# VISION-SJTU/UniDefense

Measured on AMD Instinct MI355X. Metric: images/sec fwd+bwd (256x256, EffNet-b4), higher is better.
Workload: dtype f32

## Files before the change

include/unidefense_hip.h:

```cpp
#ifndef UNIDEFENSE_HIP_H
#define UNIDEFENSE_HIP_H
#include <stdint.h>

#ifdef __cplusplus
extern "C" {
#endif

#define UD_EINVAL (-1000)

typedef void* ud_stream_t;

typedef struct {
    int N, Hin, Win, Cin, Hout, Wout, KH, KW, stride, pad_t, pad_l, transposed;
} ud_conv_geom;

typedef struct {
    const float* A; const float* B; float* C;
    int M, N, K;
    long lda, ldb, ldc;
    int a_mode, b_mode, out_mode, split_k;
    int batch; long strideA, strideB, strideC;
    ud_conv_geom g;
    double* stat_sum; double* stat_sumsq;
    int half_mask;
// ... 393 lines not shown
int ud_pj_bwd_fused_a(const float* d, const float* dp, const ud_bn_ref* bn, const float* s, const float* w, int N, int HW, int CE,
                      int CO, float* dw, double* dgate, float* part, ud_stream_t stream);
int ud_pj_bwd_fused_b(const float* d, const float* dp, const ud_bn_ref* bn, const float* s, const float* dpool, float inv_hw,
                      const float* w, int N, int HW, int CE, int CO, float* dz, double* s1, double* s2, ud_stream_t stream);
int ud_normbwd_apply_plane_half(const void* x, const void* dy, const float* keep, float inv_keep, const ud_bn_ref* bn,
                                int dy_is_dz, const double* s1, const double* s2, const double* s1_local,
                                const double* s2_local, int G, int R, int C, uint16_t* plane, long panel_stride,
                                float* inv_scale, float* dgamma, float* dbeta, ud_stream_t stream);
int ud_se_bwd_a(const double* dgate, const float* s2, const float* s1, const float* We, double* ds1_acc, float* dWe,
                float* dbe, int N, int C, int Cs, ud_stream_t stream);
int ud_se_bwd_b(const double* ds1_acc, const float* s1, const float* Wr, const double* pool, float pool_scale,
                float* dpool, float* dWr, float* dbr, int N, int C, int Cs, ud_stream_t stream);
int ud_se_scale_bwd_bn(const void* dc, const void* x, const ud_bn_ref* bn, const float* s, const float* dpool,
    float inv_hw, void* dz, double* s1, double* s2, double* ws, int G, int R, int C, int f16, ud_stream_t
    stream);
long ud_coldot_bn_eval_ws_doubles(int G, int R, int C);
int ud_coldot_bn_eval(const void* dy, const void* x, const ud_bn_ref* bn, int G, int R, int C, double* out, double* ws,
                      int f16, ud_stream_t stream);
int ud_se_scale_bwd_bn_eval(const void* dc, const void* x, const ud_bn_ref* bn, const float* s, const float* dpool,
                            float inv_hw, void* dd, int G, int R, int C, int f16, ud_stream_t stream);
int ud_bn_eval_bwd(const void* dy, const void* x, const ud_bn_ref* bn, void* dx, int G, int R, int C, int f16,
                   ud_stream_t stream);
int ud_normbwd_apply_mix(const void* x, const void* dz, const ud_bn_ref* bn, const double* s1, const double* s2,
    const double* s1_local, const double* s2_local, const void* diff, int G, int R, int C, void* dd,
    double* dalpha_acc, float* dgamma, float* dbeta, double* energy, int f16, ud_stream_t stream);
int ud_gate_grad_from_acc(const double* acc, const float* alpha, float* out, ud_stream_t stream);
int ud_bn_apply(const void* x, const ud_bn_ref* bn, void* y, int G, int R, int C, int f16, ud_stream_t stream);
int ud_dwconv_bwd_data_bn(const void* dy, const float* gate_alpha, int gate_mode, const float* wt, const void*
    add, const void* x, const ud_bn_ref* bn, void* dz, double* s1, double* s2, double* ws, int N, int H, int W,
    int C, int Ho, int Wo, int K, int stride, int pad_t, int pad_l, int f16, ud_stream_t stream);
// ... 80 lines not shown
```

unidefense_amd/csrc/fused.hip:

```cpp
#include "bnref.h"

namespace {

struct Rows {
    int r, r_end;
    long idx, step;
};
__device__ __forceinline__ Rows rows_of(const RedGeom& q, int ri, int c4) {
    Rows w;
    const int g = blockIdx.z, p = blockIdx.x;
    const int r_begin = p * q.rows_per_chunk;
    w.r_end = r_begin + q.rows_per_chunk;
    if (w.r_end > q.R) w.r_end = q.R;
    w.step = (long)q.rpi * q.C4;
    w.r = r_begin + ri;
    w.idx = (long)g * q.R * q.C4 + (long)w.r * q.C4 + c4;
    return w;
}

__device__ __forceinline__ bool is_updater(int ri) { return blockIdx.x == 0 && blockIdx.z == 0 && ri == 0; }

template <int NQ>
__device__ __forceinline__ void red_out(const RedGeom& q, int ri, bool active, int c4, double (&v)[8], double* a1,
                                        double* a2, double* part, bool per_group) {
// ... 2 lines not shown
    if (part) {
        const long o = (((long)blockIdx.z * q.P + blockIdx.x) * q.C4 + c4) * 4;
        const long plane = (long)q.G * q.P * q.C4 * 4;
#pragma unroll
        for (int e = 0; e < 4; ++e) {
            part[o + e] = v[e];
            if (NQ == 8) part[plane + o + e] = v[4 + e];
        }
    } else {
        const long o = ((long)(per_group ? blockIdx.z : 0) * q.C4 + c4) * 4;
#pragma unroll
        for (int e = 0; e < 4; ++e) {
            atomic_add_f64(a1 + o + e, v[e]);
            if (NQ == 8) atomic_add_f64(a2 + o + e, v[4 + e]);
        }
    }
}

template <typename T>
__global__ __launch_bounds__(NT) void colstats_kernel(RedGeom q, const T* __restrict__ x, double* __restrict__ sum,
                                                      double* __restrict__ sumsq, double* __restrict__ part) {
    int ri, c4;
    const bool active = thread_coords(q, ri, c4);
    const In4<T> x4{x};
    double v[8] = {0, 0, 0, 0, 0, 0, 0, 0};
    if (active) {
        Rows w = rows_of(q, ri, c4);
        for (; w.r + 3 * q.rpi < w.r_end; w.r += 4 * q.rpi, w.idx += 4 * w.step) {
            f32x4 a0 = x4[w.idx], a1 = x4[w.idx + w.step], a2 = x4[w.idx + 2 * w.step], a3 = x4[w.idx + 3 * w.step];
#pragma unroll
// ... 42 lines not shown
                });
            } else {
                const In4<T> in[1] = {x4};
                for_rows<T, 1>(w.r, w.r_end, q.rpi, w.idx, w.step, in, fin, [&](long, int, const f32x4(&t)[1]) UD_LAMBDA_INLINE {
                    const f32x4 a = bn_apply<ACT>(t[0], cb);
#pragma unroll
                    for (int e = 0; e < 4; ++e) v[e] += (double)a[e];
                    mo = fmaxf(mo, fmaxf(fmaxf(fabsf(a[0]), fabsf(a[1])), fmaxf(fabsf(a[2]), fabsf(a[3]))));
                });
            }
        });
        if (!DOT && is_updater(ri)) bn_update_running(bn, blockIdx.z, q.C4, c4);
    }
    red_out<4>(q, ri, active, c4, v, out, nullptr, part, true);
    if (!DOT) ud_absmax_commit(mo, amax);
}

__global__ __launch_bounds__(NT) void fc_fwd_d_kernel(const double* __restrict__ xsum, float xscale,
                                                      const float* __restrict__ W, const float* __restrict__ b,
                                                      float* __restrict__ y, int N, int I, int O) {
    const int wave = (blockIdx.x * NT + threadIdx.x) >> 6, lane = threadIdx.x & 63;
    if (wave >= N * O) return;
    const int n = wave / O, o = wave % O;
    float acc = 0.f;
#pragma unroll 4
    for (int i = lane; i < I; i += 64) acc += ((float)xsum[(long)n * I + i] * xscale) * W[(long)o * I + i];
    acc = ud_wave_sum(acc);
    if (lane == 0) y[(long)n * O + o] = acc + (b ? b[o] : 0.f);
}

// ... 219 lines not shown
    const In4<T> in[1] = {In4<T>{x}};
    const Out4<T> y4{y};
    const BnRaw raw = bn_issue(bn, blockIdx.z, q.C4, c4);
    Bn4 cb;
    const Rows w = rows_of(q, ri, c4);
    auto fin = [&]() UD_LAMBDA_INLINE { cb = bn_finish(bn, raw); };
    act_switch(bn.act, [&](auto ac) UD_LAMBDA_INLINE {
        constexpr int ACT = decltype(ac)::value;
        for_rows<T, 1>(w.r, w.r_end, q.rpi, w.idx, w.step, in, fin,
                       [&](long idx, int, const f32x4(&t)[1]) UD_LAMBDA_INLINE { y4.st(idx, bn_apply<ACT>(t[0], cb)); });
    });
    if (is_updater(ri)) bn_update_running(bn, blockIdx.z, q.C4, c4);
}

constexpr int kDz = -1;
template <int MODE>
__device__ __forceinline__ void dz_terms(const f32x4& a, const f32x4& d, const Bn4& cb, float sc, f32x4& dz, f32x4& xh) {
#pragma unroll
    for (int e = 0; e < 4; ++e) {
        xh[e] = (a[e] - cb.mu[e]) * cb.is[e];
        float g = d[e];
        if (MODE != kDz) {
            g = mul_rn(g, sc);
            if (MODE) g = mul_rn(g, ud_act_grad_fast(cb.ga[e] * xh[e] + cb.be[e], MODE));
        }
        dz[e] = g;
    }
}
template <typename F>
__device__ __forceinline__ void dz_switch(int dy_is_dz, int act, F&& f) {
    if (dy_is_dz) f(ActC<kDz>{});
    else act_switch(act, f);
}

template <typename T>
__global__ __launch_bounds__(NT) void normbwd_sums_kernel(RedGeom q, const T* __restrict__ x,
                                                          const T* __restrict__ dy, const float* __restrict__ keep,
                                                          float inv_keep, ud_bn_ref bn, int dy_is_dz,
                                                          double* __restrict__ s1, double* __restrict__ s2,
                                                          double* __restrict__ s3, double* __restrict__ part) {
    int ri, c4;
    const bool active = thread_coords(q, ri, c4);
    const In4<T> x4{x}, d4{dy};
    double v[8] = {0, 0, 0, 0, 0, 0, 0, 0};
    f32x4 en = {0.f, 0.f, 0.f, 0.f};
    if (active) {
        const BnRaw raw = bn_issue(bn, blockIdx.z, q.C4, c4);
// ... 26 lines not shown
        if (active && ri == 0) {
#pragma unroll
            for (int e = 0; e < 4; ++e) atomic_add_f64(s3 + (long)c4 * 4 + e, ev[e]);
        }
    }
    red_out<8>(q, ri, active, c4, v, s1, s2, part, false);
}

struct PlanesDst {
    uint16_t* buf;
    long panel, plane;
    float* inv_scale;
    const double* energy;
};

template <typename T, bool MIX, int PL = 0>
__global__ __launch_bounds__(NT) void normbwd_apply_kernel(RedGeom q, const T* __restrict__ x,
                                                           const T* __restrict__ dy, const float* __restrict__ keep,
                                                           float inv_keep, ud_bn_ref bn, int dy_is_dz,
                                                           const double* __restrict__ s1, const double* __restrict__ s2,
                                                           const double* __restrict__ s1l, const double* __restrict__ s2l,
                                                           const T* __restrict__ freq,
                                                           T* __restrict__ dx, double* __restrict__ dalpha_acc,
                                                           float* __restrict__ dgamma, float* __restrict__ dbeta,
                                                           uint32_t* __restrict__ amax, double* __restrict__ energy,
                                                           PlanesDst pd) {
    int ri, c4;
    const bool active = thread_coords(q, ri, c4);
    BnRaw raw{};
    double t1d[4] = {0, 0, 0, 0}, t2d[4] = {0, 0, 0, 0};
    float kraw = 0.f;
    if (active) {
        raw = bn_issue(bn, blockIdx.z, q.C4, c4);
#pragma unroll
        for (int e = 0; e < 4; ++e) t1d[e] = s1[c4 * 4 + e];
#pragma unroll
        for (int e = 0; e < 4; ++e) t2d[e] = s2[c4 * 4 + e];
        if (keep) kraw = keep[blockIdx.z];
    }
    float ps = 1.f;
    if constexpr (PL == 2) {
        if (blockIdx.x == 0 && blockIdx.y == 0 && blockIdx.z == 0 && threadIdx.x == 0) *pd.inv_scale = 1.f;
    }
    if constexpr (PL == 1) {
        __shared__ float pl_red[NT / 64];
        float gm = 0.f;
        for (int i = threadIdx.x; i < q.C4 * 4; i += NT) {
            const double m = bn.sum[i] * bn.inv_count;
// ... 17 lines not shown
    double acc = 0.0;
    float mo = 0.f;
    f32x4 en = {0.f, 0.f, 0.f, 0.f};
    if (active) {
        Bn4 cb;
        float sc = 1.f;
        f32x4 t1, t2, k;
        const Rows w = rows_of(q, ri, c4);
        uint16_t* po = PL ? pd.buf + (long)(c4 >> 3) * pd.panel + (c4 & 7) * 4 : nullptr;
        const int npad = (PL && c4 == q.C4 - 1) ? 7 - (c4 & 7) : 0;
        const long prow0 = (long)blockIdx.z * q.R;
        auto fin = [&]() UD_LAMBDA_INLINE {
            cb = bn_finish(bn, raw);
            if (keep) sc = kraw * inv_keep;
            k = cb.ga * cb.is;
#pragma unroll
            for (int e = 0; e < 4; ++e) {
                t1[e] = (float)t1d[e] * (float)bn.inv_count;
                t2[e] = (float)t2d[e] * (float)bn.inv_count;
            }
        };
        auto row = [&](auto mc, const f32x4& a, const f32x4& d, const f32x4* f, long idx, int r) UD_LAMBDA_INLINE {
            constexpr int MODE = decltype(mc)::value;
            f32x4 dz, xh, o;
            dz_terms<MODE>(a, d, cb, sc, dz, xh);
#pragma unroll
            for (int e = 0; e < 4; ++e) o[e] = k[e] * __builtin_fmaf(-xh[e], t2[e], dz[e] - t1[e]);
            if constexpr (PL == 2) {
                typedef unsigned short u16x4 __attribute__((ext_vector_type(4)));
                const long prow = prow0 + r;
                Quad<T>::st(reinterpret_cast<T*>(po + prow * 32), 0, o);
                for (int z = 1; z <= npad; ++z) *reinterpret_cast<u16x4*>(po + prow * 32 + 4 * z) = u16x4{0, 0, 0, 0};
            } else if constexpr (PL == 1) {
                typedef unsigned short u16x4 __attribute__((ext_vector_type(4)));
                const long prow = prow0 + r;
                uint16_t h0[4], h1[4];
#pragma unroll
                for (int e = 0; e < 4; ++e) ud_split_h2(o[e] * ps, h0[e], h1[e]);
                *reinterpret_cast<u16x4*>(po + prow * 32) = u16x4{h0[0], h0[1], h0[2], h0[3]};
                *reinterpret_cast<u16x4*>(po + prow * 32 + pd.plane) = u16x4{h1[0], h1[1], h1[2], h1[3]};
                for (int z = 1; z <= npad; ++z) {
                    *reinterpret_cast<u16x4*>(po + prow * 32 + 4 * z) = u16x4{0, 0, 0, 0};
                    *reinterpret_cast<u16x4*>(po + prow * 32 + 4 * z + pd.plane) = u16x4{0, 0, 0, 0};
                }
            } else {
                o4.st(idx, o);
                mo = fmaxf(mo, fmaxf(fmaxf(fabsf(o[0]), fabsf(o[1])), fmaxf(fabsf(o[2]), fabsf(o[3]))));
                if constexpr (MIX) {
#pragma unroll
                    for (int e = 0; e < 4; ++e) acc += (double)ud_rounded<T>(o[e]) * (double)(*f)[e];
                    en += o * o;
                }
            }
        };
        dz_switch(dy_is_dz, bn.act, [&](auto mc) UD_LAMBDA_INLINE {
            if constexpr (MIX) {
                const In4<T> in[3] = {x4, d4, fr4};
                for_rows<T, 3>(w.r, w.r_end, q.rpi, w.idx, w.step, in, fin, [&](long idx, int r, const f32x4(&t)[3]) UD_LAMBDA_INLINE {
                    row(mc, t[0], t[1], &t[2], idx, r);
                });
            } else {
                const In4<T> in[2] = {x4, d4};
                for_rows<T, 2>(w.r, w.r_end, q.rpi, w.idx, w.step, in, fin, [&](long idx, int r, const f32x4(&t)[2]) UD_LAMBDA_INLINE {
                    row(mc, t[0], t[1], nullptr, idx, r);
                });
            }
        });
        if (is_updater(ri)) {
#pragma unroll
            for (int e = 0; e < 4; ++e) {
// ... 198 lines not shown
        __syncthreads();
        if (own) {
#pragma unroll 8
            for (int n = 0; n < nn; ++n) {
                const float g = sh[sl * IP + n];
                acc += g * ud_act_fast(s1[(long)(n0 + n) * Cs + i], 1);
                accb += g;
            }
        }
    }
    if (!own) return;
    dWe[(long)c * Cs + i] = acc;
    if (i == 0) dbe[c] = accb;
}

__global__ __launch_bounds__(NT) void se_bwd_b_kernel(const double* __restrict__ ds1_acc, const float* __restrict__ s1,
                                                      const float* __restrict__ Wr, const double* __restrict__ pool,
                                                      float pool_scale, float* __restrict__ dpool,
                                                      float* __restrict__ dWr, float* __restrict__ dbr, int N, int C,
                                                      int Cs) {
    __shared__ float sh[NT];
    const int c = blockIdx.x * NT + threadIdx.x;
    if ((int)blockIdx.y < N) {
        const int n = blockIdx.y;
        if ((int)threadIdx.x < Cs)
            sh[threadIdx.x] = (float)ds1_acc[(long)n * Cs + threadIdx.x] * ud_act_grad_fast(s1[(long)n * Cs + threadIdx.x], 1);
        __syncthreads();
        if (c >= C) return;
        float acc = 0.f;
#pragma unroll 8
        for (int i = 0; i < Cs; ++i) acc += sh[i] * Wr[(long)i * C + c];
        dpool[(long)n * C + c] = acc;
        return;
    }
    const int i = blockIdx.y - N;
    if ((int)threadIdx.x < N)
        sh[threadIdx.x] = (float)ds1_acc[(long)threadIdx.x * Cs + i] * ud_act_grad_fast(s1[(long)threadIdx.x * Cs + i], 1);
    __syncthreads();
    if (blockIdx.x == 0 && threadIdx.x == 0) {
        float b = 0.f;
        for (int n = 0; n < N; ++n) b += sh[n];
        dbr[i] = b;
    }
    if (c >= C) return;
    float acc = 0.f;
#pragma unroll 8
    for (int n = 0; n < N; ++n) acc += sh[n] * ((float)pool[(long)n * C + c] * pool_scale);
// ... 390 lines not shown
    return finish_reduce(pl, 2, false, C, ws, s1, s2, s);
}

int ud_normbwd_apply(const void* x, const void* dy, const float* keep, float inv_keep, const ud_bn_ref* bn,
                     int dy_is_dz, const double* s1, const double* s2, const double* s1_local,
                     const double* s2_local, int G, int R, int C, void* dx, float* dgamma, float* dbeta, int f16,
                     uint32_t* absmax, ud_stream_t stream) {
    if (ud_bn_eval_form(bn)) return UD_EINVAL;
    if (!shape_ok(G, R, C) || !x || !dy || !bn || !s1 || !s2 || !dx || bn->G != 1) return UD_EINVAL;
    if ((dgamma || dbeta) && (!s1_local || !s2_local)) return UD_EINVAL;
    RedGeom q = geom_ew(G, R, C);
    UD_STORAGE_DISPATCH(f16, hipLaunchKernelGGL((normbwd_apply_kernel<T, false>), red_grid(q), dim3(NT), 0,
                                                (hipStream_t)stream, q, (const T*)x, (const T*)dy, keep, inv_keep, *bn,
                                                dy_is_dz, s1, s2, s1_local, s2_local, (const T*)nullptr, (T*)dx,
                                                (double*)nullptr, dgamma, dbeta, absmax, (double*)nullptr,
                                                PlanesDst{nullptr, 0, 0, nullptr, nullptr}));
    UD_LAUNCH_CHECK();
    return 0;
}

int ud_normbwd_apply_planes(const float* x, const float* dy, const float* keep, float inv_keep, const ud_bn_ref* bn,
                            int dy_is_dz, const double* s1, const double* s2, const double* s1_local,
                            const double* s2_local, const double* energy, int G, int R, int C, uint16_t* planes,
                            long panel_stride, long plane_stride, float* inv_scale, float* dgamma, float* dbeta,
                            ud_stream_t stream) {
    if (ud_bn_eval_form(bn)) return UD_EINVAL;
    if (!shape_ok(G, R, C) || !x || !dy || !bn || !s1 || !s2 || !energy || !planes || !inv_scale || bn->G != 1 || !bn->gamma)
        return UD_EINVAL;
    if ((dgamma || dbeta) && (!s1_local || !s2_local)) return UD_EINVAL;
    const long rows = (long)G * R;
    if (panel_stride < 32 * rows || plane_stride < (long)ud_cdiv(C, 32) * panel_stride) return UD_EINVAL;
    RedGeom q = geom_ew(G, R, C);
    hipLaunchKernelGGL((normbwd_apply_kernel<float, false, 1>), red_grid(q), dim3(NT), 0, (hipStream_t)stream, q, x, dy, keep,
                       inv_keep, *bn, dy_is_dz, s1, s2, s1_local, s2_local, (const float*)nullptr, (float*)nullptr,
                       (double*)nullptr, dgamma, dbeta, (uint32_t*)nullptr, (double*)nullptr,
                       PlanesDst{planes, panel_stride, plane_stride, inv_scale, energy});
    UD_LAUNCH_CHECK();
    return 0;
}

int ud_normbwd_apply_plane_half(const void* x, const void* dy, const float* keep, float inv_keep, const ud_bn_ref* bn,
                                int dy_is_dz, const double* s1, const double* s2, const double* s1_local,
                                const double* s2_local, int G, int R, int C, uint16_t* plane, long panel_stride,
                                float* inv_scale, float* dgamma, float* dbeta, ud_stream_t stream) {
    if (ud_bn_eval_form(bn)) return UD_EINVAL;
    if (!shape_ok(G, R, C) || !x || !dy || !bn || !s1 || !s2 || !plane || !inv_scale || bn->G != 1) return UD_EINVAL;
    if ((dgamma || dbeta) && (!s1_local || !s2_local)) return UD_EINVAL;
    if (panel_stride < 32L * G * R) return UD_EINVAL;
    RedGeom q = geom_ew(G, R, C);
    hipLaunchKernelGGL((normbwd_apply_kernel<_Float16, false, 2>), red_grid(q), dim3(NT), 0, (hipStream_t)stream, q,
                       (const _Float16*)x, (const _Float16*)dy, keep, inv_keep, *bn, dy_is_dz, s1, s2, s1_local, s2_local,
                       (const _Float16*)nullptr, (_Float16*)nullptr, (double*)nullptr, dgamma, dbeta, (uint32_t*)nullptr,
                       (double*)nullptr, PlanesDst{plane, panel_stride, 0, inv_scale, nullptr});
    UD_LAUNCH_CHECK();
    return 0;
}

int ud_normbwd_apply_mix(const void* x, const void* dz, const ud_bn_ref* bn, const double* s1, const double* s2,
                         const double* s1_local, const double* s2_local, const void* diff, int G, int R, int C,
                         void* dd, double* dalpha_acc, float* dgamma, float* dbeta, double* energy, int f16,
                         ud_stream_t stream) {
    if (ud_bn_eval_form(bn)) return UD_EINVAL;
    if (!shape_ok(G, R, C) || !x || !dz || !bn || !s1 || !s2 || !dd || !diff || !dalpha_acc || bn->G != 1)
        return UD_EINVAL;
    if ((dgamma || dbeta) && (!s1_local || !s2_local)) return UD_EINVAL;
    RedGeom q = make_geom_ex(G, R, C, 512, 4096, 4);
    UD_STORAGE_DISPATCH(f16, hipLaunchKernelGGL((normbwd_apply_kernel<T, true>), red_grid(q), dim3(NT), 0,
                                                (hipStream_t)stream, q, (const T*)x, (const T*)dz, (const float*)nullptr,
                                                1.f, *bn, 1, s1, s2, s1_local, s2_local, (const T*)diff, (T*)dd,
                                                dalpha_acc, dgamma, dbeta, (uint32_t*)nullptr, energy,
                                                PlanesDst{nullptr, 0, 0, nullptr, nullptr}));
    UD_LAUNCH_CHECK();
    return 0;
}

int ud_gate_grad_from_acc(const double* acc, const float* alpha, float* out, ud_stream_t stream) {
    if (!acc || !alpha || !out) return UD_EINVAL;
    hipLaunchKernelGGL(gate_grad_from_acc_kernel, dim3(1), dim3(64), 0, (hipStream_t)stream, acc, alpha, out);
    UD_LAUNCH_CHECK();
    return 0;
}

int ud_se_bwd_a(const double* dgate, const float* s2, const float* s1, const float* We, double* ds1_acc, float* dWe,
                float* dbe, int N, int C, int Cs, ud_stream_t stream) {
    if (N < 1 || C < 1 || Cs < 1 || Cs > 128 || !dgate || !s2 || !s1 || !We || !ds1_acc || (!dWe != !dbe)) return UD_EINVAL;
    hipStream_t s = (hipStream_t)stream;
// ... 4 lines not shown
        hipLaunchKernelGGL(se_bwd_a_kernel<64>, grid, dim3(NT), 0, s, dgate, s2, s1, We, ds1_acc, dWe, dbe, N, C, Cs);
    } else {
        dim3 grid((unsigned)(role1 + (wg ? ud_cdiv(C, NT / 128) : 0)));
        hipLaunchKernelGGL(se_bwd_a_kernel<128>, grid, dim3(NT), 0, s, dgate, s2, s1, We, ds1_acc, dWe, dbe, N, C, Cs);
    }
    UD_LAUNCH_CHECK();
    return 0;
}

int ud_se_bwd_b(const double* ds1_acc, const float* s1, const float* Wr, const double* pool, float pool_scale,
                float* dpool, float* dWr, float* dbr, int N, int C, int Cs, ud_stream_t stream) {
    const bool wg = dWr != nullptr;
    if (N < 1 || N > NT || C < 1 || Cs < 1 || Cs > NT || !ds1_acc || !s1 || !Wr || !dpool || (!dWr != !dbr) || (wg && !pool))
        return UD_EINVAL;
    dim3 grid((unsigned)ud_cdiv(C, NT), (unsigned)(N + (wg ? Cs : 0)));
    hipLaunchKernelGGL(se_bwd_b_kernel, grid, dim3(NT), 0, (hipStream_t)stream, ds1_acc, s1, Wr, pool, pool_scale, dpool,
                       dWr, dbr, N, C, Cs);
    UD_LAUNCH_CHECK();
    return 0;
}

int ud_se_scale_bwd_bn(const void* dc, const void* x, const ud_bn_ref* bn, const float* s, const float* dpool,
                       float inv_hw, void* dz, double* s1, double* s2, double* ws, int G, int R, int C, int f16,
                       ud_stream_t stream) {
    if (ud_bn_eval_form(bn)) return UD_EINVAL;
    if (!shape_ok(G, R, C) || !dc || !x || !bn || !s || !dpool || !dz || !s1 || !s2 || bn->G != 1) return UD_EINVAL;
    hipStream_t st = (hipStream_t)stream;
    RedPlan pl = plan_reduce(G, R, C, false, ws);
    UD_STORAGE_DISPATCH(f16, hipLaunchKernelGGL(se_scale_bwd_bn_kernel<T>, red_grid(pl.q), dim3(NT), 0, st, pl.q,
                                                (const T*)dc, (const T*)x, *bn, s, dpool, inv_hw, (T*)dz, s1, s2,
                                                pl.use_part ? ws : nullptr));
    UD_LAUNCH_CHECK();
// ... 150 lines not shown
```

unidefense_amd/kernels.py:

```python
import ctypes as C
import math
import os

import torch

from . import lib as _lib
from .config import cfg as CFG
from .devmem import Scratch, ZeroPool
from .lib import ConvGeom, GemmDesc, GemmP3Desc

_call = _lib.call
_const, _rows = _lib.const, _lib.const_rows

GEMM_PROFILE = None


def _stream():
    return C.c_void_p(torch.cuda.current_stream().cuda_stream)


def _p(t):
    if t is None:
        return None
    return C.c_void_p(t.data_ptr())
# ... 2656 lines not shown
    _act(x)
    _chk(s)
    Cc = x.shape[-1]
    pl = Planes(G * R, Cc, x, 1, False)
    _call("ud_se_scale_bn_plane_half", _p(x), C.byref(bn.ref()), _p(s), _p(pl.buf), pl.panel, _p(pl.inv), G, R, Cc, _stream())
    return pl


def coldot_bn(dy, x, bn, G, R, out):
    h = _act(dy, x)
    Cc = x.shape[-1]
    _call("ud_coldot_bn", _p(dy), _p(x), C.byref(bn.ref()), G, R, Cc, _pd(out), _fused_ws(x, G, R, Cc, True), h,
          _stream())


def fc_fwd_d(xsum, xscale, W, b, N):
    _chk(W, b)
    O, I = W.shape
    y = empty((N, O), W)
    _call("ud_fc_fwd_d", _pd(xsum), float(xscale), _p(W), _p(b), _p(y), N, I, O, _stream())
    return y


def bn_apply(x, bn, G, R, update=False):
    h = _act(x)
    y = torch.empty_like(x)
    _call("ud_bn_apply", _p(x), C.byref(bn.ref(update)), _p(y), G, R, x.shape[-1], h, _stream())
    return y


# ... 148 lines not shown
    return dz


def normbwd_apply_mix(x, dz, bn, G, R, sacc, diff, dalpha_acc, sacc_local=None, energy=None):
    h = _act(x, dz, diff)
    Cc = x.shape[-1]
    loc = sacc if sacc_local is None else sacc_local
    dd = torch.empty_like(x)
    dg = empty((Cc,), x)
    db = empty((Cc,), x)
    _call("ud_normbwd_apply_mix", _p(x), _p(dz), C.byref(bn.ref()), _pd(sacc), _pd(sacc, Cc), _pd(loc), _pd(loc, Cc),
          _p(diff), G, R, Cc, _p(dd), _pd(dalpha_acc), _p(dg), _p(db), _pd(energy) if energy is not None else None, h, _stream())
    return dd, dg, db


def gate_grad_from_acc(acc, alpha):
    out = empty((), alpha)
    _call("ud_gate_grad_from_acc", _pd(acc), _p(alpha), _p(out), _stream())
    return out


def se_bwd(dgate, s2, s1, We, Wr, pool, pool_scale, need_w=True):
    _chk(s2, s1, We, Wr)
    N, Cc = s2.shape
    Cs = s1.shape[1]
    ds1_acc = zeros64(N * Cs, s2)
    if not need_w:
        _call("ud_se_bwd_a", _pd(dgate), _p(s2), _p(s1), _p(We), _pd(ds1_acc), None, None, N, Cc, Cs, _stream())
        dpool = empty((N, Cc), s2)
        _call("ud_se_bwd_b", _pd(ds1_acc), _p(s1), _p(Wr), None, 0.0, _p(dpool), None, None, N, Cc, Cs, _stream())
        return dpool, None, None, None, None
    dWe = empty((Cc, Cs), s2)
    dbe = empty((Cc,), s2)
    _call("ud_se_bwd_a", _pd(dgate), _p(s2), _p(s1), _p(We), _pd(ds1_acc), _p(dWe), _p(dbe), N, Cc, Cs, _stream())
    dpool = empty((N, Cc), s2)
    dWr = empty((Cs, Cc), s2)
    dbr = empty((Cs,), s2)
    _call("ud_se_bwd_b", _pd(ds1_acc), _p(s1), _p(Wr), _pd(pool), float(pool_scale), _p(dpool), _p(dWr), _p(dbr), N, Cc,
          Cs, _stream())
    return dpool, dWe, dbe, dWr, dbr


def se_scale_bwd_bn(dc, x, bn, s, dpool, inv_hw, G, R, sacc):
    h = _act(dc, x)
    _chk(s, dpool)
    Cc = x.shape[-1]
    dz = torch.empty_like(x)
    _call("ud_se_scale_bwd_bn", _p(dc), _p(x), C.byref(bn.ref()), _p(s), _p(dpool), float(inv_hw), _p(dz), _pd(sacc),
          _pd(sacc, Cc), _fused_ws(x, G, R, Cc, False), G, R, Cc, h, _stream())
    return dz


# ... 308 lines not shown
```

unidefense_amd/mbconv.py:

```python
import collections
from types import SimpleNamespace

import torch

from . import kernels as K
from . import tape as T
from .config import cfg


FUSED, HALF, EVAL_NODE, OPERATORS = "fused", "half", "eval_node", "operators"
TrunkMode = collections.namedtuple("TrunkMode", "kind wt dp", defaults=(None,))


_DW_TILED = True


_DW_TILE_OVERRIDE = {}
_DW_BWD_FUSED_OVERRIDE = {}


def _dw_tile_policy(sf, k, stride, H, half):
    ov = _DW_TILE_OVERRIDE.get((bool(sf), k, stride, H, bool(half)))
    if ov is not None and _DW_TILED:
        return ov
# ... 13 lines not shown
    bwd = (k == 5 and H >= 16) or (k == 3 and 32 <= H <= 64)
    return (fwd or not sf), not sf, bwd


def _dw_bwd_fused_policy(sf, k, stride, H, half):
    if stride != 1:
        return False
    ov = _DW_BWD_FUSED_OVERRIDE.get((bool(sf), k, stride, H, bool(half)))
    if ov is not None:
        return ov
    if H <= 8:
        return k == 3 and not half
    if half:
        return True
    return not (k == 3 and H == 64)


BlockGeom = collections.namedtuple(
    "BlockGeom", "N H W Cin M k stride pt pl Ho Wo HWo Mo Ce Co Cs We Wsr Wse Wp Wf sf alpha s_f s_i")


def block_geom(blk, x):
    sp = blk.spec
    N, H, W, Cin = x.shape
    Ho, Wo = T.conv_out_hw(H, W, sp.k, sp.stride, sp.pad)
    Ce, Co, Cs = sp.cexp, sp.cout, sp.cse
    sf = sp.sf_norm is not None
    dwm = blk._depthwise_conv
    s_f, s_i = T._fft_scales(H, sp.sf_norm) if sf else (None, None)
    return BlockGeom(N, H, W, Cin, N * H * W, sp.k, sp.stride, sp.pad[2], sp.pad[0], Ho, Wo, Ho * Wo, N * Ho * Wo, Ce, Co, Cs,
# ... 232 lines not shown
        dx._ud_owned = True
        tape.add_grad(b.x, dx)


def _bwd_project(b, tape, gr):
    g, x, blk, dout = b.geo, b.x, b.blk, gr.dout
    dp_pl = K.normbwd_planes_ok(b.p4, b.pctx)
    sb2 = K.zeros64((3 if dp_pl == 1 else 2) * g.Co, x)
    K.normbwd_sums(b.p4, dout, b.keep, b.inv_keep, b.bn2, False, g.N, g.HWo, sb2)
    loc2 = b.dp.reduce(sb2, keep_local=True)
    gr.dp2, dp_amax, dg2, db2 = _normbwd_to_gemm(b.pctx, dp_pl, b.p4, dout, b.keep, b.inv_keep, b.bn2, False, g.N, g.HWo, sb2, loc2)
    tape.add_param_grad(blk._bn2.weight, dg2)
    tape.add_param_grad(blk._bn2.bias, db2)
    gr.pj_fused = not dp_pl and b.pctx.plans is None and K.project_bwd_fused_ok(b.d, g.Wp, g.HWo)
    assert gr.pj_fused or b.pctx.x is not None, "the fused project forward kept no gated tensor: its backward must be the fused one"
    gr.dgate = K.zeros64(g.N * g.Ce, x)
    if gr.pj_fused:
        gr.dc = None
        dWp = K.project_bwd_fused_a(b.d, b.bn1, b.s2, gr.dp2, g.Wp, g.N, g.HWo, gr.dgate)
    else:
        dc, dWp = K.spectral_bwd(b.pctx, gr.dp2, dy_absmax=dp_amax)
        gr.dc = dc.view(g.N, g.Ho, g.Wo, g.Ce)
        K.coldot_bn(gr.dc, b.d, b.bn1, g.N, g.HWo, gr.dgate)
    tape.add_param_grad(blk._project_conv.weight, dWp)


def _bwd_se(b, tape, gr):
    g, blk = b.geo, b.blk
    dpool, dWe2, dbe2, dWr, dbr = K.se_bwd(gr.dgate, b.s2, b.s1, g.Wse, g.Wsr, b.pool, 1.0 / g.HWo)
    tape.add_param_grad(blk._se_expand.weight, dWe2)
    tape.add_param_grad(blk._se_expand.bias, dbe2)
    tape.add_param_grad(blk._se_reduce.weight, dWr)
    tape.add_param_grad(blk._se_reduce.bias, dbr)
    gr.sb1 = K.zeros64(2 * g.Ce, b.x)
    if gr.pj_fused:
        gr.dz1 = K.project_bwd_fused_b(b.d, b.bn1, b.s2, dpool, 1.0 / g.HWo, gr.dp2, g.Wp, g.N, g.HWo, gr.sb1)
    else:
        gr.dz1 = K.se_scale_bwd_bn(gr.dc, b.d, b.bn1, b.s2, dpool, 1.0 / g.HWo, g.N, g.HWo, gr.sb1)
    gr.loc1 = b.dp.reduce(gr.sb1, keep_local=True)


def _bwd_bn1(b, tape, gr):
    g, x, blk, d = b.geo, b.x, b.blk, b.d
    gr.g_alpha, gr.g_mode, gr.da_f, gr.dxf = None, 0, None, None
    if not g.sf:
        gr.g_sp, dg1, db1 = K.normbwd_apply(d, gr.dz1, None, 1.0, b.bn1, True, g.N, g.HWo, gr.sb1, gr.loc1)
    else:
        alpha, sctx = g.alpha, b.sctx
        if g.stride == 1:
            dacc = K.zeros64(64, x)
            dyf_pl = sctx.plans is not None and K.rfft2_planes_ok(d, None)
            en = K.zeros64(g.Ce, x) if dyf_pl else None
            dd, dg1, db1 = K.normbwd_apply_mix(d, gr.dz1, b.bn1, g.N, g.HWo, gr.sb1, b.fr, dacc, gr.loc1, energy=en)
            form = _PLANES if dyf_pl else _PLANE_HALF if (sctx.plans is not None and K.rfft2_plane_half_ok(dd)) else _ROWS
            bound = {"energy": en} if dyf_pl else {}
            dyf, _, dalpha = _rfft2_as(form, dd, g.s_i, 2.0, gate_alpha=alpha, gate_mode=1, gate_acc=dacc, **bound)
            tape.add_param_grad(alpha, dalpha)
            gr.g_sp, gr.g_alpha, gr.g_mode = dd, alpha, 2
        else:
            dd, dg1, db1 = K.normbwd_apply(d, gr.dz1, None, 1.0, b.bn1, True, g.N, g.HWo, gr.sb1, gr.loc1)
            gr.g_sp, dfr, dalpha = K.sfmix_bwd(b.spat, b.fr, alpha, dd, True)
            tape.add_param_grad(alpha, dalpha)
            dyf = K.rfft2(dfr, g.s_i, 2.0, want_absmax=True)
        dyf2, dyf_amax = _gemm_dy(sctx, dyf, dd)
        dxf, dWf = K.spectral_bwd(sctx, dyf2, dy_absmax=dyf_amax)
        tape.add_param_grad(blk._depthwise_conv.freq_conv.weight, dWf)
        gr.dxf = dxf.view(b.xf_shape)
        if not b.irdw:
            gr.da_f = K.irfft2(gr.dxf, g.s_f, 0.5)
    tape.add_param_grad(blk._bn1.weight, dg1)
    tape.add_param_grad(blk._bn1.bias, db1)


def _expand_planes_route(b):
    if b.e is None or b.lazy_in is not None:
# ... 199 lines not shown
```

Baseline: 1401.

## Fold SE-scale BN1 backward statistics into the coldot pass and SE-bwd kernel

In the non-fused project path, the gate dot-product pass now also accumulates the per-(n,c) partial sums needed for the BN1 backward statistics. The SE backward kernel then combines these with the sigmoid gate and dpool into the BN sums, which removes the separate se_scale_bwd_bn pass over the full activation and the materialised dz1 tensor. The BN1 apply kernels recompute dz on the fly from dc, the gate and dpool. The cost is a heavier reduction kernel with 20 double accumulators per thread, 5x larger gate buffers, and extra atomics.

```diff
diff --git a/include/unidefense_hip.h b/include/unidefense_hip.h
--- a/include/unidefense_hip.h
+++ b/include/unidefense_hip.h
@@ -431,6 +431,18 @@
 int ud_se_scale_bwd_bn(const void* dc, const void* x, const ud_bn_ref* bn, const float* s, const float* dpool,
     float inv_hw, void* dz, double* s1, double* s2, double* ws, int G, int R, int C, int f16, ud_stream_t
     stream);
+int ud_coldot_bn_se(const void* dy, const void* x, const ud_bn_ref* bn, int G, int R, int C, double* out, int f16,
+                    ud_stream_t stream);
+int ud_se_bwd_b_bn(const double* ds1_acc, const float* s1, const float* Wr, const double* pool, float pool_scale,
+                   float* dpool, float* dWr, float* dbr, const float* s2, const double* dots, float inv_hw, double* bs1,
+                   double* bs2, int N, int C, int Cs, ud_stream_t stream);
+int ud_normbwd_apply_se(const void* x, const void* dc, const ud_bn_ref* bn, const float* s, const float* dpool, float inv_hw,
+                        const double* s1, const double* s2, const double* s1_local, const double* s2_local, int G, int R,
+                        int C, void* dx, float* dgamma, float* dbeta, int f16, uint32_t* absmax, ud_stream_t stream);
+int ud_normbwd_apply_mix_se(const void* x, const void* dc, const ud_bn_ref* bn, const float* s, const float* dpool,
+                            float inv_hw, const double* s1, const double* s2, const double* s1_local,
+                            const double* s2_local, const void* diff, int G, int R, int C, void* dd, double* dalpha_acc,
+                            float* dgamma, float* dbeta, double* energy, int f16, ud_stream_t stream);
 long ud_coldot_bn_eval_ws_doubles(int G, int R, int C);
 int ud_coldot_bn_eval(const void* dy, const void* x, const ud_bn_ref* bn, int G, int R, int C, double* out, double* ws,
                       int f16, ud_stream_t stream);
diff --git a/unidefense_amd/csrc/fused.hip b/unidefense_amd/csrc/fused.hip
--- a/unidefense_amd/csrc/fused.hip
+++ b/unidefense_amd/csrc/fused.hip
@@ -40,6 +40,25 @@
             atomic_add_f64(a1 + o + e, v[e]);
             if (NQ == 8) atomic_add_f64(a2 + o + e, v[4 + e]);
         }
+    }
+}
+template <int NQ>
+__device__ __forceinline__ void red_out_spread(const RedGeom& q, int ri, bool active, int c4, double (&v)[NQ], double* out) {
+    __shared__ double sm[NQ * NT];
+    if (active) {
+#pragma unroll
+        for (int i = 0; i < NQ; ++i) sm[i * NT + threadIdx.x] = v[i];
+    }
+    __syncthreads();
+    if (!active) return;
+    const int col = (int)threadIdx.x - ri * q.CW;
+    const long plane = (long)q.G * q.C4 * 4;
+    const long o = ((long)blockIdx.z * q.C4 + c4) * 4;
+    for (int i = ri; i < NQ; i += q.rpi) {
+        const double* s = sm + i * NT + col;
+        double t = 0.0;
+        for (int r = 0; r < q.rpi; ++r) t += s[r * q.CW];
+        atomic_add_f64(out + (i >> 2) * plane + o + (i & 3), t);
     }
 }
 
@@ -112,6 +131,43 @@
     }
     red_out<4>(q, ri, active, c4, v, out, nullptr, part, true);
     if (!DOT) ud_absmax_commit(mo, amax);
+}
+
+template <typename T>
+__global__ __launch_bounds__(NT) void coldot_bn_se_kernel(RedGeom q, const T* __restrict__ x, const T* __restrict__ dy,
+                                                          ud_bn_ref bn, double* __restrict__ out) {
+    int ri, c4;
+    const bool active = thread_coords(q, ri, c4);
+    const In4<T> x4{x}, d4{dy};
+    double v[20];
+#pragma unroll
+    for (int i = 0; i < 20; ++i) v[i] = 0.0;
+    if (active) {
+        const BnRaw raw = bn_issue(bn, blockIdx.z, q.C4, c4);
+        Bn4 cb;
+        const Rows w = rows_of(q, ri, c4);
+        auto fin = [&]() UD_LAMBDA_INLINE { cb = bn_finish(bn, raw); };
+        act_switch(bn.act, [&](auto ac) UD_LAMBDA_INLINE {
+            constexpr int ACT = decltype(ac)::value;
+            const In4<T> in[2] = {x4, d4};
+            for_rows<T, 2>(w.r, w.r_end, q.rpi, w.idx, w.step, in, fin, [&](long, int, const f32x4(&t)[2]) UD_LAMBDA_INLINE {
+                const f32x4 a = bn_apply<ACT>(t[0], cb);
+#pragma unroll
+                for (int e = 0; e < 4; ++e) {
+                    const float xh = (t[0][e] - cb.mu[e]) * cb.is[e];
+                    const float ap = ACT ? ud_act_grad_fast(cb.ga[e] * xh + cb.be[e], ACT) : 1.f;
+                    const double dyd = (double)t[1][e], xhd = (double)xh, apd = (double)ap;
+                    const double u = (double)mul_rn(t[1][e], ap);
+                    v[e] += dyd * (double)a[e];
+                    v[4 + e] += u;
+                    v[8 + e] += u * xhd;
+                    v[12 + e] += apd;
+                    v[16 + e] += apd * xhd;
+                }
+            });
+        });
+    }
+    red_out_spread<20>(q, ri, active, c4, v, out);
 }
 
 __global__ __launch_bounds__(NT) void fc_fwd_d_kernel(const double* __restrict__ xsum, float xscale,
@@ -361,23 +417,35 @@
 }
 
 constexpr int kDz = -1;
+constexpr int kSe = 8;
+struct SeGate { f32x4 g, p; };
 template <int MODE>
-__device__ __forceinline__ void dz_terms(const f32x4& a, const f32x4& d, const Bn4& cb, float sc, f32x4& dz, f32x4& xh) {
+__device__ __forceinline__ void dz_terms(const f32x4& a, const f32x4& d, const Bn4& cb, float sc, f32x4& dz, f32x4& xh,
+                                         const SeGate& se = SeGate{}) {
 #pragma unroll
     for (int e = 0; e < 4; ++e) {
         xh[e] = (a[e] - cb.mu[e]) * cb.is[e];
         float g = d[e];
-        if (MODE != kDz) {
+        if constexpr (MODE >= kSe) {
+            g = g * se.g[e] + se.p[e];
+            if (MODE - kSe) g *= ud_act_grad_fast(cb.ga[e] * xh[e] + cb.be[e], MODE - kSe);
+        } else if (MODE != kDz) {
             g = mul_rn(g, sc);
             if (MODE) g = mul_rn(g, ud_act_grad_fast(cb.ga[e] * xh[e] + cb.be[e], MODE));
         }
         dz[e] = g;
     }
 }
-template <typename F>
+template <bool SE = false, typename F>
 __device__ __forceinline__ void dz_switch(int dy_is_dz, int act, F&& f) {
-    if (dy_is_dz) f(ActC<kDz>{});
-    else act_switch(act, f);
+    if constexpr (SE) {
+        if (act == 1) f(ActC<kSe + 1>{});
+        else if (act == 2) f(ActC<kSe + 2>{});
+        else f(ActC<kSe>{});
+    } else {
+        if (dy_is_dz) f(ActC<kDz>{});
+        else act_switch(act, f);
+    }
 }
 
 template <typename T>
@@ -434,7 +502,12 @@
     const double* energy;
 };
 
-template <typename T, bool MIX, int PL = 0>
+struct SeSrc {
+    const float* s;
+    const float* dpool;
+    float inv_hw;
+};
+template <typename T, bool MIX, int PL = 0, bool SE = false>
 __global__ __launch_bounds__(NT) void normbwd_apply_kernel(RedGeom q, const T* __restrict__ x,
                                                            const T* __restrict__ dy, const float* __restrict__ keep,
                                                            float inv_keep, ud_bn_ref bn, int dy_is_dz,
@@ -444,14 +517,19 @@
                                                            T* __restrict__ dx, double* __restrict__ dalpha_acc,
                                                            float* __restrict__ dgamma, float* __restrict__ dbeta,
                                                            uint32_t* __restrict__ amax, double* __restrict__ energy,
-                                                           PlanesDst pd) {
+                                                           PlanesDst pd, SeSrc se) {
     int ri, c4;
     const bool active = thread_coords(q, ri, c4);
     BnRaw raw{};
     double t1d[4] = {0, 0, 0, 0}, t2d[4] = {0, 0, 0, 0};
     float kraw = 0.f;
+    SeGate sg{};
     if (active) {
         raw = bn_issue(bn, blockIdx.z, q.C4, c4);
+        if constexpr (SE) {
+            sg.g = reinterpret_cast<const f32x4*>(se.s)[(long)blockIdx.z * q.C4 + c4];
+            sg.p = reinterpret_cast<const f32x4*>(se.dpool)[(long)blockIdx.z * q.C4 + c4];
+        }
 #pragma unroll
         for (int e = 0; e < 4; ++e) t1d[e] = s1[c4 * 4 + e];
 #pragma unroll
@@ -499,6 +577,11 @@
             cb = bn_finish(bn, raw);
             if (keep) sc = kraw * inv_keep;
             k = cb.ga * cb.is;
+            if constexpr (SE) {
+                sg.p = sg.p * se.inv_hw;
+#pragma unroll
+                for (int e = 0; e < 4; ++e) sg.g[e] = ud_sigmoid_fast(sg.g[e]);
+            }
 #pragma unroll
             for (int e = 0; e < 4; ++e) {
                 t1[e] = (float)t1d[e] * (float)bn.inv_count;
@@ -508,7 +591,7 @@
         auto row = [&](auto mc, const f32x4& a, const f32x4& d, const f32x4* f, long idx, int r) UD_LAMBDA_INLINE {
             constexpr int MODE = decltype(mc)::value;
             f32x4 dz, xh, o;
-            dz_terms<MODE>(a, d, cb, sc, dz, xh);
+            dz_terms<MODE>(a, d, cb, sc, dz, xh, sg);
 #pragma unroll
             for (int e = 0; e < 4; ++e) o[e] = k[e] * __builtin_fmaf(-xh[e], t2[e], dz[e] - t1[e]);
             if constexpr (PL == 2) {
@@ -538,7 +621,7 @@
                 }
             }
         };
-        dz_switch(dy_is_dz, bn.act, [&](auto mc) UD_LAMBDA_INLINE {
+        dz_switch<SE>(dy_is_dz, bn.act, [&](auto mc) UD_LAMBDA_INLINE {
             if constexpr (MIX) {
                 const In4<T> in[3] = {x4, d4, fr4};
                 for_rows<T, 3>(w.r, w.r_end, q.rpi, w.idx, w.step, in, fin, [&](long idx, int r, const f32x4(&t)[3]) UD_LAMBDA_INLINE {
@@ -767,11 +850,19 @@
     if (i == 0) dbe[c] = accb;
 }
 
+struct SeBnFold {
+    const float* s2;
+    const double* dots;
+    float inv_hw;
+    double* bs1;
+    double* bs2;
+};
+template <bool BN>
 __global__ __launch_bounds__(NT) void se_bwd_b_kernel(const double* __restrict__ ds1_acc, const float* __restrict__ s1,
                                                       const float* __restrict__ Wr, const double* __restrict__ pool,
                                                       float pool_scale, float* __restrict__ dpool,
                                                       float* __restrict__ dWr, float* __restrict__ dbr, int N, int C,
-                                                      int Cs) {
+                                                      int Cs, SeBnFold f) {
     __shared__ float sh[NT];
     const int c = blockIdx.x * NT + threadIdx.x;
     if ((int)blockIdx.y < N) {
@@ -780,10 +871,22 @@
             sh[threadIdx.x] = (float)ds1_acc[(long)n * Cs + threadIdx.x] * ud_act_grad_fast(s1[(long)n * Cs + threadIdx.x], 1);
         __syncthreads();
         if (c >= C) return;
+        const long o = (long)n * C + c, plane = (long)N * C;
+        float gs = 0.f;
+        double a1 = 0.0, a2 = 0.0, b1 = 0.0, b2 = 0.0;
+        if constexpr (BN) {
+            gs = f.s2[o];
+            a1 = f.dots[plane + o], a2 = f.dots[2 * plane + o], b1 = f.dots[3 * plane + o], b2 = f.dots[4 * plane + o];
+        }
         float acc = 0.f;
 #pragma unroll 8
         for (int i = 0; i < Cs; ++i) acc += sh[i] * Wr[(long)i * C + c];
-        dpool[(long)n * C + c] = acc;
+        dpool[o] = acc;
+        if constexpr (BN) {
+            const double g = (double)ud_sigmoid_fast(gs), p = (double)mul_rn(acc, f.inv_hw);
+            atomic_add_f64(f.bs1 + c, g * a1 + p * b1);
+            atomic_add_f64(f.bs2 + c, g * a2 + p * b2);
+        }
         return;
     }
     const int i = blockIdx.y - N;
@@ -1204,7 +1307,7 @@
                                                 (hipStream_t)stream, q, (const T*)x, (const T*)dy, keep, inv_keep, *bn,
                                                 dy_is_dz, s1, s2, s1_local, s2_local, (const T*)nullptr, (T*)dx,
                                                 (double*)nullptr, dgamma, dbeta, absmax, (double*)nullptr,
-                                                PlanesDst{nullptr, 0, 0, nullptr, nullptr}));
+                                                PlanesDst{nullptr, 0, 0, nullptr, nullptr}, SeSrc{}));
     UD_LAUNCH_CHECK();
     return 0;
 }
@@ -1224,7 +1327,7 @@
     hipLaunchKernelGGL((normbwd_apply_kernel<float, false, 1>), red_grid(q), dim3(NT), 0, (hipStream_t)stream, q, x, dy, keep,
                        inv_keep, *bn, dy_is_dz, s1, s2, s1_local, s2_local, (const float*)nullptr, (float*)nullptr,
                        (double*)nullptr, dgamma, dbeta, (uint32_t*)nullptr, (double*)nullptr,
-                       PlanesDst{planes, panel_stride, plane_stride, inv_scale, energy});
+                       PlanesDst{planes, panel_stride, plane_stride, inv_scale, energy}, SeSrc{});
     UD_LAUNCH_CHECK();
     return 0;
 }
@@ -1241,7 +1344,7 @@
     hipLaunchKernelGGL((normbwd_apply_kernel<_Float16, false, 2>), red_grid(q), dim3(NT), 0, (hipStream_t)stream, q,
                        (const _Float16*)x, (const _Float16*)dy, keep, inv_keep, *bn, dy_is_dz, s1, s2, s1_local, s2_local,
                        (const _Float16*)nullptr, (_Float16*)nullptr, (double*)nullptr, dgamma, dbeta, (uint32_t*)nullptr,
-                       (double*)nullptr, PlanesDst{plane, panel_stride, 0, inv_scale, nullptr});
+                       (double*)nullptr, PlanesDst{plane, panel_stride, 0, inv_scale, nullptr}, SeSrc{});
     UD_LAUNCH_CHECK();
     return 0;
 }
@@ -1259,7 +1362,7 @@
                                                 (hipStream_t)stream, q, (const T*)x, (const T*)dz, (const float*)nullptr,
                                                 1.f, *bn, 1, s1, s2, s1_local, s2_local, (const T*)diff, (T*)dd,
                                                 dalpha_acc, dgamma, dbeta, (uint32_t*)nullptr, energy,
-                                                PlanesDst{nullptr, 0, 0, nullptr, nullptr}));
+                                                PlanesDst{nullptr, 0, 0, nullptr, nullptr}, SeSrc{}));
     UD_LAUNCH_CHECK();
     return 0;
 }
@@ -1294,8 +1397,65 @@
     if (N < 1 || N > NT || C < 1 || Cs < 1 || Cs > NT || !ds1_acc || !s1 || !Wr || !dpool || (!dWr != !dbr) || (wg && !pool))
         return UD_EINVAL;
     dim3 grid((unsigned)ud_cdiv(C, NT), (unsigned)(N + (wg ? Cs : 0)));
-    hipLaunchKernelGGL(se_bwd_b_kernel, grid, dim3(NT), 0, (hipStream_t)stream, ds1_acc, s1, Wr, pool, pool_scale, dpool,
-                       dWr, dbr, N, C, Cs);
+    hipLaunchKernelGGL(se_bwd_b_kernel<false>, grid, dim3(NT), 0, (hipStream_t)stream, ds1_acc, s1, Wr, pool, pool_scale, dpool,
+                       dWr, dbr, N, C, Cs, SeBnFold{});
+    UD_LAUNCH_CHECK();
+    return 0;
+}
+
+int ud_coldot_bn_se(const void* dy, const void* x, const ud_bn_ref* bn, int G, int R, int C, double* out, int f16,
+                    ud_stream_t stream) {
+    if (ud_bn_eval_form(bn)) return UD_EINVAL;
+    if (!shape_ok(G, R, C) || !x || !dy || !bn || !out || bn->G != 1 || f16) return UD_EINVAL;
+    RedPlan pl = plan_reduce(G, R, C, true, nullptr);
+    hipLaunchKernelGGL(coldot_bn_se_kernel<float>, red_grid(pl.q), dim3(NT), 0, (hipStream_t)stream, pl.q, (const float*)x,
+                       (const float*)dy, *bn, out);
+    UD_LAUNCH_CHECK();
+    return 0;
+}
+
+int ud_se_bwd_b_bn(const double* ds1_acc, const float* s1, const float* Wr, const double* pool, float pool_scale,
+                   float* dpool, float* dWr, float* dbr, const float* s2, const double* dots, float inv_hw, double* bs1,
+                   double* bs2, int N, int C, int Cs, ud_stream_t stream) {
+    const bool wg = dWr != nullptr;
+    if (N < 1 || N > NT || C < 1 || Cs < 1 || Cs > NT || !ds1_acc || !s1 || !Wr || !dpool || (!dWr != !dbr) || (wg && !pool))
+        return UD_EINVAL;
+    if (!s2 || !dots || !bs1 || !bs2) return UD_EINVAL;
+    dim3 grid((unsigned)ud_cdiv(C, NT), (unsigned)(N + (wg ? Cs : 0)));
+    hipLaunchKernelGGL(se_bwd_b_kernel<true>, grid, dim3(NT), 0, (hipStream_t)stream, ds1_acc, s1, Wr, pool, pool_scale, dpool,
+                       dWr, dbr, N, C, Cs, SeBnFold{s2, dots, inv_hw, bs1, bs2});
+    UD_LAUNCH_CHECK();
+    return 0;
+}
+
+int ud_normbwd_apply_se(const void* x, const void* dc, const ud_bn_ref* bn, const float* s, const float* dpool, float inv_hw,
+                        const double* s1, const double* s2, const double* s1_local, const double* s2_local, int G, int R,
+                        int C, void* dx, float* dgamma, float* dbeta, int f16, uint32_t* absmax, ud_stream_t stream) {
+    if (ud_bn_eval_form(bn)) return UD_EINVAL;
+    if (!shape_ok(G, R, C) || !x || !dc || !bn || !s || !dpool || !s1 || !s2 || !dx || bn->G != 1 || f16) return UD_EINVAL;
+    if ((dgamma || dbeta) && (!s1_local || !s2_local)) return UD_EINVAL;
+    RedGeom q = geom_ew(G, R, C);
+    hipLaunchKernelGGL((normbwd_apply_kernel<float, false, 0, true>), red_grid(q), dim3(NT), 0, (hipStream_t)stream, q,
+                       (const float*)x, (const float*)dc, (const float*)nullptr, 1.f, *bn, 0, s1, s2, s1_local, s2_local,
+                       (const float*)nullptr, (float*)dx, (double*)nullptr, dgamma, dbeta, absmax, (double*)nullptr,
+                       PlanesDst{nullptr, 0, 0, nullptr, nullptr}, SeSrc{s, dpool, inv_hw});
+    UD_LAUNCH_CHECK();
+    return 0;
+}
+
+int ud_normbwd_apply_mix_se(const void* x, const void* dc, const ud_bn_ref* bn, const float* s, const float* dpool,
+                            float inv_hw, const double* s1, const double* s2, const double* s1_local,
+                            const double* s2_local, const void* diff, int G, int R, int C, void* dd, double* dalpha_acc,
+                            float* dgamma, float* dbeta, double* energy, int f16, ud_stream_t stream) {
+    if (ud_bn_eval_form(bn)) return UD_EINVAL;
+    if (!shape_ok(G, R, C) || !x || !dc || !bn || !s || !dpool || !s1 || !s2 || !dd || !diff || !dalpha_acc || bn->G != 1 || f16)
+        return UD_EINVAL;
+    if ((dgamma || dbeta) && (!s1_local || !s2_local)) return UD_EINVAL;
+    RedGeom q = make_geom_ex(G, R, C, 512, 4096, 4);
+    hipLaunchKernelGGL((normbwd_apply_kernel<float, true, 0, true>), red_grid(q), dim3(NT), 0, (hipStream_t)stream, q,
+                       (const float*)x, (const float*)dc, (const float*)nullptr, 1.f, *bn, 0, s1, s2, s1_local, s2_local,
+                       (const float*)diff, (float*)dd, dalpha_acc, dgamma, dbeta, (uint32_t*)nullptr, energy,
+                       PlanesDst{nullptr, 0, 0, nullptr, nullptr}, SeSrc{s, dpool, inv_hw});
     UD_LAUNCH_CHECK();
     return 0;
 }
diff --git a/unidefense_amd/kernels.py b/unidefense_amd/kernels.py
--- a/unidefense_amd/kernels.py
+++ b/unidefense_amd/kernels.py
@@ -2694,6 +2694,12 @@
           _stream())
 
 
+def coldot_bn_se(dy, x, bn, G, R, out):
+    _chk(dy, x)
+    assert x.dtype == torch.float32 and dy.dtype == torch.float32 and out.numel() >= 5 * G * x.shape[-1]
+    _call("ud_coldot_bn_se", _p(dy), _p(x), C.byref(bn.ref()), G, R, x.shape[-1], _pd(out), 0, _stream())
+
+
 def fc_fwd_d(xsum, xscale, W, b, N):
     _chk(W, b)
     O, I = W.shape
@@ -2872,13 +2878,41 @@
     return dd, dg, db
 
 
+def normbwd_apply_se(x, dc, bn, s, dpool, inv_hw, G, R, sacc, sacc_local=None):
+    _chk(x, dc, s, dpool)
+    assert x.dtype == torch.float32 and dc.dtype == torch.float32
+    Cc = x.shape[-1]
+    loc = sacc if sacc_local is None else sacc_local
+    dx = torch.empty_like(x)
+    dg = empty((Cc,), x)
+    db = empty((Cc,), x)
+    _call("ud_normbwd_apply_se", _p(x), _p(dc), C.byref(bn.ref()), _p(s), _p(dpool), float(inv_hw), _pd(sacc), _pd(sacc, Cc),
+          _pd(loc), _pd(loc, Cc), G, R, Cc, _p(dx), _p(dg), _p(db), 0, None, _stream())
+    dx._ud_absmax = None
+    return dx, dg, db
+
+
+def normbwd_apply_mix_se(x, dc, bn, s, dpool, inv_hw, G, R, sacc, diff, dalpha_acc, sacc_local=None, energy=None):
+    _chk(x, dc, diff, s, dpool)
+    assert x.dtype == torch.float32 and dc.dtype == torch.float32 and diff.dtype == torch.float32
+    Cc = x.shape[-1]
+    loc = sacc if sacc_local is None else sacc_local
+    dd = torch.empty_like(x)
+    dg = empty((Cc,), x)
+    db = empty((Cc,), x)
+    _call("ud_normbwd_apply_mix_se", _p(x), _p(dc), C.byref(bn.ref()), _p(s), _p(dpool), float(inv_hw), _pd(sacc), _pd(sacc, Cc),
+          _pd(loc), _pd(loc, Cc), _p(diff), G, R, Cc, _p(dd), _pd(dalpha_acc), _p(dg), _p(db),
+          _pd(energy) if energy is not None else None, 0, _stream())
+    return dd, dg, db
+
+
 def gate_grad_from_acc(acc, alpha):
     out = empty((), alpha)
     _call("ud_gate_grad_from_acc", _pd(acc), _p(alpha), _p(out), _stream())
     return out
 
 
-def se_bwd(dgate, s2, s1, We, Wr, pool, pool_scale, need_w=True):
+def se_bwd(dgate, s2, s1, We, Wr, pool, pool_scale, need_w=True, fold=None):
     _chk(s2, s1, We, Wr)
     N, Cc = s2.shape
     Cs = s1.shape[1]
@@ -2894,6 +2928,12 @@
     dpool = empty((N, Cc), s2)
     dWr = empty((Cs, Cc), s2)
     dbr = empty((Cs,), s2)
+    if fold is not None:
+        dots, inv_hw, sacc = fold
+        assert dots.numel() >= 5 * N * Cc and sacc.numel() >= 2 * Cc
+        _call("ud_se_bwd_b_bn", _pd(ds1_acc), _p(s1), _p(Wr), _pd(pool), float(pool_scale), _p(dpool), _p(dWr), _p(dbr), _p(s2),
+              _pd(dots), float(inv_hw), _pd(sacc), _pd(sacc, Cc), N, Cc, Cs, _stream())
+        return dpool, dWe, dbe, dWr, dbr
     _call("ud_se_bwd_b", _pd(ds1_acc), _p(s1), _p(Wr), _pd(pool), float(pool_scale), _p(dpool), _p(dWr), _p(dbr), N, Cc,
           Cs, _stream())
     return dpool, dWe, dbe, dWr, dbr
diff --git a/unidefense_amd/mbconv.py b/unidefense_amd/mbconv.py
--- a/unidefense_amd/mbconv.py
+++ b/unidefense_amd/mbconv.py
@@ -51,6 +51,18 @@
     if half:
         return True
     return not (k == 3 and H == 64)
+
+
+_SE_BN1_FOLD_OVERRIDE = {}
+
+
+def _se_bn1_fold_policy(sf, stride, Ho, Ce, half):
+    if half:
+        return False
+    ov = _SE_BN1_FOLD_OVERRIDE.get((bool(sf), stride, Ho, Ce))
+    if ov is not None:
+        return ov
+    return True
 
 
 BlockGeom = collections.namedtuple(
@@ -313,51 +325,73 @@
     tape.add_param_grad(blk._bn2.bias, db2)
     gr.pj_fused = not dp_pl and b.pctx.plans is None and K.project_bwd_fused_ok(b.d, g.Wp, g.HWo)
     assert gr.pj_fused or b.pctx.x is not None, "the fused project forward kept no gated tensor: its backward must be the fused one"
-    gr.dgate = K.zeros64(g.N * g.Ce, x)
+    gr.se_dots = None
     if gr.pj_fused:
         gr.dc = None
+        gr.dgate = K.zeros64(g.N * g.Ce, x)
         dWp = K.project_bwd_fused_a(b.d, b.bn1, b.s2, gr.dp2, g.Wp, g.N, g.HWo, gr.dgate)
     else:
         dc, dWp = K.spectral_bwd(b.pctx, gr.dp2, dy_absmax=dp_amax)
         gr.dc = dc.view(g.N, g.Ho, g.Wo, g.Ce)
-        K.coldot_bn(gr.dc, b.d, b.bn1, g.N, g.HWo, gr.dgate)
+        if _se_bn1_fold_policy(g.sf, g.stride, g.Ho, g.Ce, b.d.dtype != torch.float32 or dc.dtype != torch.float32):
+            gr.se_dots = K.zeros64(5 * g.N * g.Ce, x)
+            gr.dgate = gr.se_dots[:g.N * g.Ce]
+            K.coldot_bn_se(gr.dc, b.d, b.bn1, g.N, g.HWo, gr.se_dots)
+        else:
+            gr.dgate = K.zeros64(g.N * g.Ce, x)
+            K.coldot_bn(gr.dc, b.d, b.bn1, g.N, g.HWo, gr.dgate)
     tape.add_param_grad(blk._project_conv.weight, dWp)
 
 
 def _bwd_se(b, tape, gr):
     g, blk = b.geo, b.blk
-    dpool, dWe2, dbe2, dWr, dbr = K.se_bwd(gr.dgate, b.s2, b.s1, g.Wse, g.Wsr, b.pool, 1.0 / g.HWo)
+    gr.sb1 = K.zeros64(2 * g.Ce, b.x)
+    fold = (gr.se_dots, 1.0 / g.HWo, gr.sb1) if gr.se_dots is not None else None
+    dpool, dWe2, dbe2, dWr, dbr = K.se_bwd(gr.dgate, b.s2, b.s1, g.Wse, g.Wsr, b.pool, 1.0 / g.HWo, fold=fold)
     tape.add_param_grad(blk._se_expand.weight, dWe2)
     tape.add_param_grad(blk._se_expand.bias, dbe2)
     tape.add_param_grad(blk._se_reduce.weight, dWr)
     tape.add_param_grad(blk._se_reduce.bias, dbr)
-    gr.sb1 = K.zeros64(2 * g.Ce, b.x)
-    if gr.pj_fused:
+    gr.dpool = dpool
+    if fold is not None:
+        gr.dz1 = None
+    elif gr.pj_fused:
         gr.dz1 = K.project_bwd_fused_b(b.d, b.bn1, b.s2, dpool, 1.0 / g.HWo, gr.dp2, g.Wp, g.N, g.HWo, gr.sb1)
     else:
         gr.dz1 = K.se_scale_bwd_bn(gr.dc, b.d, b.bn1, b.s2, dpool, 1.0 / g.HWo, g.N, g.HWo, gr.sb1)
     gr.loc1 = b.dp.reduce(gr.sb1, keep_local=True)
+
+
+def _bn1_apply(b, gr):
+    g = b.geo
+    if gr.dz1 is None:
+        return K.normbwd_apply_se(b.d, gr.dc, b.bn1, b.s2, gr.dpool, 1.0 / g.HWo, g.N, g.HWo, gr.sb1, gr.loc1)
+    return K.normbwd_apply(b.d, gr.dz1, None, 1.0, b.bn1, True, g.N, g.HWo, gr.sb1, gr.loc1)
 
 
 def _bwd_bn1(b, tape, gr):
     g, x, blk, d = b.geo, b.x, b.blk, b.d
     gr.g_alpha, gr.g_mode, gr.da_f, gr.dxf = None, 0, None, None
     if not g.sf:
-        gr.g_sp, dg1, db1 = K.normbwd_apply(d, gr.dz1, None, 1.0, b.bn1, True, g.N, g.HWo, gr.sb1, gr.loc1)
+        gr.g_sp, dg1, db1 = _bn1_apply(b, gr)
     else:
         alpha, sctx = g.alpha, b.sctx
         if g.stride == 1:
             dacc = K.zeros64(64, x)
             dyf_pl = sctx.plans is not None and K.rfft2_planes_ok(d, None)
             en = K.zeros64(g.Ce, x) if dyf_pl else None
-            dd, dg1, db1 = K.normbwd_apply_mix(d, gr.dz1, b.bn1, g.N, g.HWo, gr.sb1, b.fr, dacc, gr.loc1, energy=en)
+            if gr.dz1 is None:
+                dd, dg1, db1 = K.normbwd_apply_mix_se(d, gr.dc, b.bn1, b.s2, gr.dpool, 1.0 / g.HWo, g.N, g.HWo, gr.sb1, b.fr, dacc,
+                                                      gr.loc1, energy=en)
+            else:
+                dd, dg1, db1 = K.normbwd_apply_mix(d, gr.dz1, b.bn1, g.N, g.HWo, gr.sb1, b.fr, dacc, gr.loc1, energy=en)
             form = _PLANES if dyf_pl else _PLANE_HALF if (sctx.plans is not None and K.rfft2_plane_half_ok(dd)) else _ROWS
             bound = {"energy": en} if dyf_pl else {}
             dyf, _, dalpha = _rfft2_as(form, dd, g.s_i, 2.0, gate_alpha=alpha, gate_mode=1, gate_acc=dacc, **bound)
             tape.add_param_grad(alpha, dalpha)
             gr.g_sp, gr.g_alpha, gr.g_mode = dd, alpha, 2
         else:
-            dd, dg1, db1 = K.normbwd_apply(d, gr.dz1, None, 1.0, b.bn1, True, g.N, g.HWo, gr.sb1, gr.loc1)
+            dd, dg1, db1 = _bn1_apply(b, gr)
             gr.g_sp, dfr, dalpha = K.sfmix_bwd(b.spat, b.fr, alpha, dd, True)
             tape.add_param_grad(alpha, dalpha)
             dyf = K.rfft2(dfr, g.s_i, 2.0, want_absmax=True)
```

After: 1422, median of 6. 1.5% higher.
